# fnzhan/Neural-Gauge-Fields

Measured on AMD Instinct MI355X. Metric: Mray/sec (800x800 lego-style frame, 192 samples/ray), higher is better.
Workload: dtype f32; 1 GPU; TriPlane 800x800 frame, S=192, preset R1 (seeded random planes 256^2, dense density preset), gauge on, white_bg; samples_per_ray=192, bake_density=1, bake_color=1, launcher=none (single process)

## Files before the change

### neural-gauge-fields_amd/csrc/ngf_field.hip

```cpp
#include <map>
#include <mutex>
#include <utility>

#include "ngf_host.hpp"
#include "ngf_infoinv.hpp"
#include "ngf_pack.hpp"
#include "ngf_render.hpp"
#include "ngf_alpha.hpp"
#ifdef NGF_EXPERIMENTS
#include "ngf_render_pc.hpp"
#include "ngf_stage.hpp"
#endif

using namespace ngf;

static thread_local char g_err[512] = "";

int ngf::fail(int code, const char *fmt, ...)
{
    va_list ap;
    va_start(ap, fmt);
    vsnprintf(g_err, sizeof(g_err), fmt, ap);
    va_end(ap);
    return code;
}

static std::atomic<int> g_knob[ngf::KNOB_COUNT];
static const char *const g_knob_name[ngf::KNOB_COUNT] = {"tile_w", "split", "waves", "nstep", "profile", "ablate", "uv_tiles", "kernel", "stage", "poison", "grid", "xcd", "tail", "ord_rows", "ord_px", "train_dwg", "pairpack"};
static bool g_knob_init = [] { for (auto &k : g_knob) k.store(-1); return true; }();

int ngf::knob(int id) { return g_knob[id].load(std::memory_order_relaxed); }

hipError_t ngf::ensure_dynamic_lds(const void *kernel, size_t bytes)
{
    static std::mutex mu;
    static std::map<std::pair<int, const void *>, size_t> done;
    int dev = 0;
    hipError_t e = hipGetDevice(&dev);
    if (e != hipSuccess) return e;
    std::lock_guard<std::mutex> lock(mu);
    size_t &have = done[{dev, kernel}];
    if (have >= bytes && have != 0) return hipSuccess;
    e = hipFuncSetAttribute(kernel, hipFuncAttributeMaxDynamicSharedMemorySize, (int)bytes);
    if (e == hipSuccess) have = bytes;
    return e;
}

__global__ void __launch_bounds__(1024) dirty_lds_kernel(unsigned pattern, int words, int spin)
{
    extern __shared__ unsigned dirty_smem[];
    for (int i = threadIdx.x; i < words; i += blockDim.x) dirty_smem[i] = pattern;
    __syncthreads();
    const unsigned long long t0 = __builtin_readcyclecounter();
    while (__builtin_readcyclecounter() - t0 < (unsigned long long)spin) __builtin_amdgcn_s_sleep(8);
    if (dirty_smem[(threadIdx.x * 97) % words] != pattern) __builtin_trap();
}

int ngf::poison_lds(hipStream_t st)
{
    if (knob(KNOB_POISON) < 0 || !(knob(KNOB_POISON) & 1)) return NGF_OK;
    constexpr int kBytes = 160 * 1024;
    static int cus = 0;
    if (!cus) {
        int dev = 0;
        hipDeviceProp_t prop;
        HIP_TRY(hipGetDevice(&dev));
        HIP_TRY(hipGetDeviceProperties(&prop, dev));
        cus = prop.multiProcessorCount;
    }
    HIP_TRY(ensure_dynamic_lds(reinterpret_cast<const void *>(dirty_lds_kernel), kBytes));
    hipLaunchKernelGGL(dirty_lds_kernel, dim3(2 * cus), dim3(1024), kBytes, st, kPoisonPattern, kBytes / 4, 40000);
    HIP_TRY(hipGetLastError());
    return NGF_OK;
}

int ngf::poison_alloc(void *p, size_t bytes, hipStream_t st)
{
    if (knob(KNOB_POISON) < 0 || !(knob(KNOB_POISON) & 2) || !p) return NGF_OK;
    HIP_TRY(hipMemsetD32Async((hipDeviceptr_t)p, (int)kPoisonPattern, bytes / 4, st));
    return NGF_OK;
}

extern "C" int ngf_debug_dirty_lds(void *hip_stream)
{
    const int old = g_knob[ngf::KNOB_POISON].load();
    g_knob[ngf::KNOB_POISON].store(1);
    const int rc = ngf::poison_lds((hipStream_t)hip_stream);
    g_knob[ngf::KNOB_POISON].store(old);
    return rc;
}

__global__ void xcd_histogram_kernel(unsigned *out)
{
    if (threadIdx.x == 0) atomicAdd(out + xcd_id(), 1u);
    const unsigned long long t0 = __builtin_readcyclecounter();
    while (__builtin_readcyclecounter() - t0 < 20000ull) __builtin_amdgcn_s_sleep(8);
}
extern "C" int ngf_debug_xcd_histogram(unsigned *out8, int32_t workgroups, void *hip_stream)
{
    if (!out8 || workgroups <= 0) return fail(NGF_E_ARG, "ngf_debug_xcd_histogram: bad argument");
    HIP_TRY(hipMemsetAsync(out8, 0, 8 * sizeof(unsigned), (hipStream_t)hip_stream));
    hipLaunchKernelGGL(xcd_histogram_kernel, dim3(workgroups), dim3(768), 0, (hipStream_t)hip_stream, out8);
    HIP_TRY(hipGetLastError());
    return NGF_OK;
}

extern "C" int ngf_debug_set(const char *name, int32_t value)
{
    if (!name) return fail(NGF_E_ARG, "ngf_debug_set: null name");
    for (int k = 0; k < ngf::KNOB_COUNT; ++k)
        if (!strcmp(name, g_knob_name[k])) { g_knob[k].store(value); return NGF_OK; }
    return fail(NGF_E_ARG, "ngf_debug_set: unknown knob '%s'", name);
}

extern "C" int32_t ngf_debug_get(const char *name)
{
    if (name)
        for (int k = 0; k < ngf::KNOB_COUNT; ++k)
            if (!strcmp(name, g_knob_name[k])) return g_knob[k].load();
    return -1;
}

struct ngf_field {
    int32_t model = 0, flags = 0, plane_c = 0, dens_dim = 0, app = 0;
    float *tex[9] = {nullptr, nullptr, nullptr, nullptr, nullptr, nullptr, nullptr, nullptr, nullptr};
    float *blob = nullptr;
    float *basis_pack = nullptr;
    double *w1pd_tmp = nullptr;
    float *w1p_tmp = nullptr;
    uint8_t *mask = nullptr;
    uint8_t *mask_cells = nullptr;
    uint8_t *mask_any = nullptr, *mask_clear = nullptr, *mask_clear4 = nullptr;
    unsigned int *counters = nullptr;
    mutable std::atomic<unsigned> next_counter{0};
    RenderArgs proto;
    int64_t bytes = 0;
    int num_cus = 256;
    std::vector<std::pair<void *, size_t>> allocs;
    int dev = 0;
    mutable std::mutex use_mu;
    mutable std::vector<hipStream_t> streams;
    mutable std::atomic<void *> last_stream{(void *)(intptr_t)-1};
};

static inline void field_use(const ngf_field *f, hipStream_t st)
{
    if (f->last_stream.load(std::memory_order_relaxed) == (void *)st) return;
    std::lock_guard<std::mutex> lk(f->use_mu);
    bool known = false;
    for (hipStream_t s : f->streams) known |= s == st;
    if (!known) f->streams.push_back(st);
    f->last_stream.store((void *)st, std::memory_order_relaxed);
}

extern "C" int64_t ngf_debug_packed_plane_floats(int32_t H, int32_t W, int32_t nc, int32_t pair)
{
    if (H < 1 || W < 1 || nc < 1) return -1;
    return (int64_t)packed_plane_floats(H, W, nc, pair != 0);
}

template <int LOG>
__global__ void __launch_bounds__(64) mask_block_any_kernel(const uint8_t *__restrict__ cells, int D, int H, int W, int bH, int bW, uint8_t *__restrict__ any)
{
    constexpr int B = 1 << LOG;
    const int b = blockIdx.x, X = b % bW, Y = (b / bW) % bH, Z = b / (bW * bH);
    const int z = Z * B - 16 + ((int)threadIdx.x >> LOG), y = Y * B - 16 + ((int)threadIdx.x & (B - 1));
    unsigned acc = 0;
    if ((int)threadIdx.x < B * B && z >= 0 && z <= D && y >= 0 && y <= H) {
        const uint8_t *row = cells + ((size_t)z * (H + 1) + y) * (W + 1);
#pragma unroll
        for (int t = 0; t < B; ++t) {
            const int x = X * B - 16 + t;
            if (x >= 0 && x <= W) acc |= row[x];
        }
    }
    const unsigned long long m = __ballot(acc != 0);
    if (threadIdx.x == 0) any[b] = m ? 1 : 0;
}

__global__ void __launch_bounds__(256) mask_block_clear_kernel(const uint8_t *__restrict__ any, int cD, int cH, int cW, uint8_t *__restrict__ clear)
{
    const int b = blockIdx.x * blockDim.x + threadIdx.x;
    if (b >= cD * cH * cW) return;
    const int X = b % cW, Y = (b / cW) % cH, Z = b / (cW * cH);
    unsigned acc = 0;
    for (int dz = -1; dz <= 1; ++dz)
        for (int dy = -1; dy <= 1; ++dy)
            for (int dx = -1; dx <= 1; ++dx) {
                const int x = X + dx, y = Y + dy, z = Z + dz;
                if (x >= 0 && x < cW && y >= 0 && y < cH && z >= 0 && z < cD) acc |= any[(z * cH + y) * cW + x];
            }
    clear[b] = acc ? 0 : 1;
}

__global__ void bake_density_kernel(const float *__restrict__ src, int H, int W, int nc, const float *__restrict__ wd,
                                    float *__restrict__ dst, int pair)
{
    const size_t total = (size_t)(H + 2) * (W + 2);
    for (size_t i = (size_t)blockIdx.x * blockDim.x + threadIdx.x; i < total; i += (size_t)gridDim.x * blockDim.x) {
        const int x = (int)(i % (W + 2)), y = (int)(i / (W + 2));
        double v = 0.0;
        if (x >= 1 && x <= W && y >= 1 && y <= H)
// ... 744 lines not shown
{
    int64_t r[4] = {0, 0, 0, 0};
    int sh[4] = {0, 0, 0, 0};
    const int nseg = make_tile_plan(n, wide, resident, tail16 >= 0 ? tail16 : kTailDefault16, r, sh);
    for (int k = 0; k < 4; ++k) { seg_rays[k] = k < nseg ? r[k] : 0; seg_shift[k] = k < nseg ? sh[k] : 0; }
    return nseg;
}

template <typename K>
static int launch_render(K kernel, K kernel_split, K kernel_prod, const ngf_field *f, RenderArgs &A, int threads, size_t lds_bytes, hipStream_t st, int wide_tile)
{
    const unsigned slot = f->next_counter.fetch_add(1) % kCounters;
    A.tile_counter = f->counters + (size_t)slot * kQueueHeads;
    if (int rc = poison_lds(st)) return rc;
    const int waves = threads / kWave;
    const int cus = knob(KNOB_GRID) > 0 && knob(KNOB_GRID) < f->num_cus ? knob(KNOB_GRID) : f->num_cus;
    const int64_t resident = (int64_t)cus * waves;
    int64_t seg_rays[4] = {0, 0, 0, 0};
    int seg_shift[4] = {0, 0, 0, 0};
    int nseg = 1;
    bool split = kernel_split != nullptr;
    if (knob(KNOB_SPLIT) >= 0) split = knob(KNOB_SPLIT) != 0 && kernel_split;
    const int forced = knob(KNOB_TILE_W);
    auto shift_of = [](int w) { int sft = 0; while ((1 << sft) < w) ++sft; return sft; };
    if (forced >= 0 || !split) {
        int tw = forced >= 0 ? forced : 64;
        if (tw != 64 && tw != 32 && tw != 16 && tw != 8 && tw != 4 && tw != 2 && tw != 1) return fail(NGF_E_ARG, "knob tile_w must be 64, 32, 16, 8, 4, 2 or 1");
        if (knob(KNOB_SPLIT) < 0) split = tw < 64 && kernel_split;
        if (tw < 4 && !split) return fail(NGF_E_ARG, "tiles of 2 or 1 rays exist in the split kernel only");
        seg_rays[0] = A.n; seg_shift[0] = shift_of(tw);
    } else {
        nseg = make_tile_plan(A.n, wide_tile, resident, knob(KNOB_TAIL) >= 0 ? knob(KNOB_TAIL) : kTailDefault16, seg_rays, seg_shift);
    }
    A.tile_shift = seg_shift[0];
    A.tile_w = 1 << seg_shift[0];
    int64_t tiles = 0, ray0 = 0;
    for (int k = 0; k < 4; ++k) {
        const int sft = k < nseg ? seg_shift[k] : seg_shift[nseg - 1];
        const int64_t r = k < nseg ? seg_rays[k] : 0;
        A.seg_shift[k] = sft;
        A.seg_ray0[k] = ray0;
        tiles += (r + (1 << sft) - 1) >> sft;
        ray0 += r;
        if (k < 3) {
            if (tiles >= ((int64_t)1 << 32)) return fail(NGF_E_ARG, "render launch of %lld tiles: split the ray list", (long long)tiles);
            A.seg_end[k] = (uint32_t)tiles;
        }
    }
    {
        const int64_t row_w = A.ord_tpr;
        A.ord_n = A.ord_tpr = A.ord_bw = A.ord_bh = 0;
        const int sft0 = seg_shift[0];
        if (split && row_w > 0 && (row_w & ((1 << sft0) - 1)) == 0 && (seg_rays[0] >> sft0) < ((int64_t)1 << 31)) {
            const int64_t tpr = row_w >> sft0, rows = seg_rays[0] / row_w;
            int64_t bh = knob(KNOB_ORD_ROWS) > 0 ? knob(KNOB_ORD_ROWS) : 80;
            int64_t bw = (knob(KNOB_ORD_PX) > 0 ? knob(KNOB_ORD_PX) : 80) >> sft0;
            if (bw < 1) bw = 1;
            if (bw > tpr) bw = tpr;
            if (knob(KNOB_ORD_ROWS) != 0 && tpr > bw && rows >= 2 && bh >= 2) {
                if (bh > rows) bh = rows;
                A.ord_tpr = (uint32_t)tpr; A.ord_bw = (uint32_t)bw; A.ord_bh = (uint32_t)bh;
                A.ord_n = (uint32_t)((rows / bh) * bh * tpr);
            }
        }
    }
    K k = split ? kernel_split : kernel;
#if defined(NGF_EXP_DUMP) || defined(NGF_EXP_TIMELINE)
    if (split && kernel_prod) k = kernel_prod;
#else
    if (split && kernel_prod && !A.dbg_weight && !A.dbg_sigma && !A.stats && !A.skip_rgb && !A.ablate) k = kernel_prod;
#endif
    HIP_TRY(ensure_dynamic_lds(reinterpret_cast<const void *>(k), lds_bytes));
    if (tiles >= ((int64_t)1 << 32)) return fail(NGF_E_ARG, "render launch of %lld tiles: split the ray list", (long long)tiles);
    A.tiles = (uint32_t)tiles;
    A.xcd_queues = knob(KNOB_XCD) > 0 ? 8 : 1;
    int64_t grid = tiles < f->num_cus ? tiles : f->num_cus;
    if (knob(KNOB_GRID) > 0 && grid > knob(KNOB_GRID)) grid = knob(KNOB_GRID);
    if (grid < 1) grid = 1;
    const int64_t per_wg = (tiles + grid - 1) / grid;
    A.waves_active = per_wg < waves ? (int)per_wg : waves;
    A.queue_waves = (uint32_t)grid;
    hipLaunchKernelGGL(k, dim3((unsigned)grid), dim3(threads), lds_bytes, st, A);
    HIP_TRY(hipGetLastError());
    return NGF_OK;
}

template <typename P>
static int launch_policy(const ngf_field *f, RenderArgs &A, hipStream_t st)
{
    if constexpr (shared_gauge<P>::value) {
        if (!A.gauge_same) return launch_policy<GaugeAny<P>>(f, A, st);
    }
    const size_t lds = ((size_t)((A.blob_floats + 3) & ~3) + P::WAVES * wave_lds_floats<P>()) * sizeof(float);
    if (lds > 160 * 1024) return fail(NGF_E_ARG, "this waves-per-CU setting needs %zu bytes of LDS (> 160 KiB)", lds);
    constexpr int wide = P::INFOINV ? 16 : 8;
    using KP = decltype(&render_kernel<P, false>);
    if constexpr (P::NSTEP == 1 && P::PROD) return launch_render<KP>(render_kernel<P, false>, render_kernel<P, true>, render_kernel<P, true, false>, f, A, P::WAVES * kWave, lds, st, wide);
    else if constexpr (P::NSTEP == 1) return launch_render<KP>(render_kernel<P, false>, render_kernel<P, true>, nullptr, f, A, P::WAVES * kWave, lds, st, wide);
    else return launch_render<KP>(render_kernel<P, false>, nullptr, nullptr, f, A, P::WAVES * kWave, lds, st, wide);
}

#ifdef NGF_EXPERIMENTS
template <typename P, int NM, int NS, int TW>
static int launch_pc(const ngf_field *f, RenderArgs &A, hipStream_t st)
{
    if constexpr (shared_gauge<P>::value) {
        if (!A.gauge_same) return launch_pc<GaugeAny<P>, NM, NS, TW>(f, A, st);
    }
    const size_t lds = ((size_t)((A.blob_floats + 3) & ~3) + PcLds<NM>::TOTAL) * sizeof(float);
    if (lds > 160 * 1024) return fail(NGF_E_ARG, "the specialised kernel needs %zu bytes of LDS (> 160 KiB)", lds);
    const unsigned slot = f->next_counter.fetch_add(1) % kCounters;
    A.tile_counter = f->counters + (size_t)slot * kQueueHeads;
    HIP_TRY(hipMemsetAsync(A.tile_counter, 0, kQueueHeads * sizeof(unsigned), st));
    if (int rc = poison_lds(st)) return rc;
    A.xcd_queues = 1;
    A.tile_w = TW;
    A.tile_shift = TW == 8 ? 3 : 2;
    auto k = render_pc_kernel<P, NM, NS, TW>;
    HIP_TRY(ensure_dynamic_lds(reinterpret_cast<const void *>(k), lds));
    const int64_t tiles = (A.n + TW - 1) / TW;
    int64_t grid = (tiles + NM - 1) / NM;
    if (grid > f->num_cus) grid = f->num_cus;
    if (grid < 1) grid = 1;
    hipLaunchKernelGGL(k, dim3((unsigned)grid), dim3((NM + NS) * kWave), lds, st, A);
    HIP_TRY(hipMemsetAsync(A.tile_counter, 0, kQueueHeads * sizeof(unsigned), st));
    HIP_TRY(hipGetLastError());
    return NGF_OK;
}
#endif

template <bool BD, bool BC>
static int launch_triplane(const ngf_field *f, RenderArgs &A, hipStream_t st)
{
#ifndef NGF_EXPERIMENTS
    if (knob(KNOB_KERNEL) > 0 || knob(KNOB_STAGE) > 0 || knob(KNOB_PROFILE) > 0 || knob(KNOB_NSTEP) > 1 || (knob(KNOB_WAVES) >= 0 && knob(KNOB_WAVES) != 12))
        return fail(NGF_E_UNSUPPORTED, "knobs kernel / stage / profile / nstep / waves select experiment kernels: load libngf_hip_exp.so (built with -DNGF_EXPERIMENTS)");
    if constexpr (BD) {
        if (A.mask.coarse) return launch_policy<MaskSkip<TriPlanePolicy<BD, BC, 12, 1>>>(f, A, st);
    }
    return launch_policy<TriPlanePolicy<BD, BC, 12, 1>>(f, A, st);
#else
    int kernel = knob(KNOB_KERNEL) >= 0 ? knob(KNOB_KERNEL) : 0;
    if (A.dbg_weight || A.skip_rgb || knob(KNOB_NSTEP) > 1 || (knob(KNOB_PROFILE) > 0 && knob(KNOB_KERNEL) != 1)) kernel = 0;
    if (knob(KNOB_TILE_W) > 8 || knob(KNOB_SPLIT) == 0) kernel = 0;
    if (kernel == 1 && knob(KNOB_PROFILE) > 0) {
        if constexpr (!BC) {
            using PP = TriPlanePolicy<BD, false, 12, 1, true>;
            return knob(KNOB_WAVES) == 88 ? launch_pc<PP, 8, 8, 8>(f, A, st) : launch_pc<PP, 12, 4, 8>(f, A, st);
        }
    }
    if (kernel == 1) {
        using P = TriPlanePolicy<BD, BC, 12, 1>;
        int tw = A.n < 40 * (int64_t)f->num_cus * 12 ? 4 : 8;
        if (knob(KNOB_TILE_W) == 4 || knob(KNOB_TILE_W) == 8) tw = knob(KNOB_TILE_W);
        const int w = knob(KNOB_WAVES) >= 0 ? knob(KNOB_WAVES) : 124;
        switch (w) {
        case 124: return tw == 8 ? launch_pc<P, 12, 4, 8>(f, A, st) : launch_pc<P, 12, 4, 4>(f, A, st);
        case 88: return tw == 8 ? launch_pc<P, 8, 8, 8>(f, A, st) : launch_pc<P, 8, 8, 4>(f, A, st);
        case 84: return tw == 8 ? launch_pc<P, 8, 4, 8>(f, A, st) : launch_pc<P, 8, 4, 4>(f, A, st);
        case 128: return launch_pc<P, 12, 4, 8>(f, A, st);
        default: return fail(NGF_E_ARG, "specialised kernel: knob waves must be 124, 88 or 84");
        }
    }
    int w = 12, ns = 1;
    if (knob(KNOB_WAVES) >= 0) w = knob(KNOB_WAVES);
    if (knob(KNOB_NSTEP) >= 0) ns = knob(KNOB_NSTEP);
    if (ns == 2) {
        if (w == 8) return launch_policy<TriPlanePolicy<BD, BC, 8, 2>>(f, A, st);
        return fail(NGF_E_ARG, "knob nstep = 2 is built for waves = 8 only");
    }
    if (knob(KNOB_STAGE) > 0 && !A.dbg_weight && !A.skip_rgb) {
        if constexpr (!BD && !BC) {
            if (w == 8) return launch_policy<TriPlaneStagedPolicy<8>>(f, A, st);
            if (w == 12) return launch_policy<TriPlaneStagedPolicy<12>>(f, A, st);
            return fail(NGF_E_ARG, "knob stage: waves must be 8 (gauge + density strips) or 12 (gauge strips)");
        }
    }
    if (knob(KNOB_PROFILE) > 0) {
        if constexpr (!BC) return launch_policy<TriPlanePolicy<BD, false, 12, 1, true>>(f, A, st);
    }
    switch (w) {
    case 8: return launch_policy<TriPlanePolicy<BD, BC, 8, 1>>(f, A, st);
    case 12:
        if constexpr (BD) {
            if (A.mask.coarse) return launch_policy<MaskSkip<TriPlanePolicy<BD, BC, 12, 1>>>(f, A, st);
        }
        return launch_policy<TriPlanePolicy<BD, BC, 12, 1>>(f, A, st);
    case 16: return launch_policy<TriPlanePolicy<BD, BC, 16, 1>>(f, A, st);
    default: return fail(NGF_E_ARG, "knob waves must be 8, 12 or 16");
    }
#endif
}

static int render_common(const ngf_field *f, RenderArgs &A, hipStream_t st)
{
    field_use(f, st);
    if (f->model == NGF_MODEL_INFOINV) {
        const bool wide = knob(KNOB_TILE_W) > 16 || knob(KNOB_SPLIT) == 0;
        if (f->flags & NGF_F_SPLIT_BF16) {
            if (wide) return fail(NGF_E_ARG, "InfoInv NGF_F_SPLIT_BF16 renders with split tiles of at most 16 rays");
            return A.mask.coarse ? launch_policy<MaskSkip<InfoInvSplitPolicy>>(f, A, st) : launch_policy<InfoInvSplitPolicy>(f, A, st);
        }
        if (wide) return launch_policy<InfoInvWidePolicy>(f, A, st);
        return A.mask.coarse ? launch_policy<MaskSkip<InfoInvPolicy>>(f, A, st) : launch_policy<InfoInvPolicy>(f, A, st);
    }
    if (f->flags & NGF_F_NO_FOLD) return launch_policy<TriPlaneNoFoldPolicy>(f, A, st);
    if ((f->flags & NGF_F_SPLIT_BF16) && (f->flags & NGF_F_BAKE_COLOR)) return A.mask.coarse ? launch_policy<MaskSkip<TriPlaneBakedBf16Policy>>(f, A, st) : launch_policy<TriPlaneBakedBf16Policy>(f, A, st);
    if (f->flags & NGF_F_SPLIT_BF16) {
        if (knob(KNOB_TILE_W) > 8 || knob(KNOB_SPLIT) == 0) return fail(NGF_E_ARG, "NGF_F_SPLIT_BF16 renders with split tiles of 4 or 8 rays");
#ifdef NGF_EXPERIMENTS
        if (knob(KNOB_WAVES) == 12)
            return (f->flags & NGF_F_BAKE_DENSITY) ? launch_policy<TriPlaneBf16Policy<true, 12>>(f, A, st) : launch_policy<TriPlaneBf16Policy<false, 12>>(f, A, st);
#endif
        return (f->flags & NGF_F_BAKE_DENSITY) ? launch_policy<TriPlaneBf16Policy<true, 8>>(f, A, st) : launch_policy<TriPlaneBf16Policy<false, 8>>(f, A, st);
    }
    const bool bd = f->flags & NGF_F_BAKE_DENSITY, bc = f->flags & NGF_F_BAKE_COLOR;
    if (bd) return bc ? launch_triplane<true, true>(f, A, st) : launch_triplane<true, false>(f, A, st);
    return bc ? launch_triplane<false, true>(f, A, st) : launch_triplane<false, false>(f, A, st);
}

extern "C" int ngf_field_render(const ngf_field *f, const float *rays, int64_t n, int32_t n_samples, int32_t white_bg,
                                int32_t mode, const float *jitter, float *rgb, float *depth, uint64_t *stats, void *hip_stream)
{
    if (!f || !rays || !rgb || !depth) return fail(NGF_E_ARG, "ngf_field_render: null argument");
    if (n < 0 || n_samples <= 0) return fail(NGF_E_ARG, "ngf_field_render: n=%lld n_samples=%d", (long long)n, n_samples);
    if (n == 0) return NGF_OK;
    RenderArgs A = f->proto;
    A.rays = rays; A.jitter = jitter; A.rgb = rgb; A.depth = depth; A.n = n; A.S = n_samples;
    A.white_bg = white_bg ? 1 : 0; A.mode = mode ? 1 : 0; A.stats = (unsigned long long *)stats;
    if (knob(KNOB_ABLATE) > 0) A.ablate = knob(KNOB_ABLATE);
    return render_common(f, A, (hipStream_t)hip_stream);
}

extern "C" int ngf_field_render_image(const ngf_field *f, const float *rays, int64_t n, int32_t row_width, int32_t n_samples, int32_t white_bg,
                                      int32_t mode, const float *jitter, float *rgb, float *depth, uint64_t *stats, void *hip_stream)
{
    if (!f || !rays || !rgb || !depth) return fail(NGF_E_ARG, "ngf_field_render_image: null argument");
    if (n < 0 || n_samples <= 0) return fail(NGF_E_ARG, "ngf_field_render_image: n=%lld n_samples=%d", (long long)n, n_samples);
    if (n == 0) return NGF_OK;
    RenderArgs A = f->proto;
    A.rays = rays; A.jitter = jitter; A.rgb = rgb; A.depth = depth; A.n = n; A.S = n_samples;
    A.white_bg = white_bg ? 1 : 0; A.mode = mode ? 1 : 0; A.stats = (unsigned long long *)stats;
    if (knob(KNOB_ABLATE) > 0) A.ablate = knob(KNOB_ABLATE);
    A.ord_tpr = row_width > 0 && (int64_t)row_width < n && f->model == NGF_MODEL_TRIPLANE ? (uint32_t)row_width : 0u;
    return render_common(f, A, (hipStream_t)hip_stream);
}

extern "C" int ngf_field_march(const ngf_field *f, const float *rays, int64_t n, int32_t n_samples, int32_t mode,
                               const float *jitter, float *sigma, float *weight, void *hip_stream)
{
    if (!f || !rays || !sigma || !weight) return fail(NGF_E_ARG, "ngf_field_march: null argument");
    if (n <= 0 || n_samples <= 0) return fail(NGF_E_ARG, "ngf_field_march: n=%lld n_samples=%d", (long long)n, n_samples);
    hipStream_t st = (hipStream_t)hip_stream;
    float *scratch = nullptr;
    HIP_TRY(hipMallocAsync((void **)&scratch, (size_t)n * 4 * sizeof(float), st));
    RenderArgs A = f->proto;
    A.rays = rays; A.jitter = jitter; A.rgb = scratch; A.depth = scratch + 3 * n; A.n = n; A.S = n_samples;
    A.white_bg = 0; A.mode = mode ? 1 : 0; A.skip_rgb = 1; A.dbg_sigma = sigma; A.dbg_weight = weight;
    int rc = render_common(f, A, st);
    (void)hipFreeAsync(scratch, st);
    return rc;
}

extern "C" int ngf_field_decode_rgb(const ngf_field *f, const float *coords, const float *dirs, int64_t n, int32_t mode,
                                    float *rgb, void *hip_stream)
{
    if (!f || !coords || !dirs || !rgb) return fail(NGF_E_ARG, "ngf_field_decode_rgb: null argument");
    if (n <= 0) return fail(NGF_E_ARG, "ngf_field_decode_rgb: n=%lld", (long long)n);
    hipStream_t st = (hipStream_t)hip_stream;
    field_use(f, st);
// ... 130 lines not shown
```

### neural-gauge-fields_amd/csrc/ngf_render.hpp

```cpp
#pragma once
#include <cstddef>
#include <type_traits>

#include "ngf_device.hpp"
#include "ngf_shade16.hpp"
#include "ngf_shade_bf16.hpp"

namespace ngf {


template <typename P> constexpr int wave_lds_floats() { return P::RING * kRecFloats + P::BATCH * 4 + P::VFEAT_FLOATS + P::STAGE_FLOATS; }

__device__ __forceinline__ void view_inputs(const float d[3], float v[16])
{
    v[0] = d[0]; v[1] = d[1]; v[2] = d[2];
#pragma unroll
    for (int k = 0; k < 3; ++k) {
        sincos_small(d[k], v[3 + 2 * k], v[9 + 2 * k]);
        sincos_small(d[k] * 2.0f, v[4 + 2 * k], v[10 + 2 * k]);
    }
    v[15] = 0.0f;
}

__device__ __forceinline__ void view_inputs_tile(const float d[3], float *dst, int seg, int K)
// ... 60 lines not shown
        Bil b = bil_setup<BAKED>(t[2 * p], t[2 * p + 1], tx);
        if (cells) cells[p] = b;
        if (BAKED && PAIR) {
            const f32x4_a8 q = *tex_at<f32x4_a8>(tx.p, (uint32_t)b.idx * 2u);
            f += bil_mix(b, q[0], q[2], q[1], q[3]);
        } else if (BAKED) {
            const float *q = tex_at<float>(tx.p, (uint32_t)b.idx), *q1 = tex_at<float>(tx.p, (uint32_t)(b.idx + tx.stride));
            f += bil_mix(b, q[0], q[1], q1[0], q1[1]);
        } else {
            const f32x4 *q00 = tex_at<f32x4>(tx.p, (uint32_t)b.idx * 16u);
            const f32x4 *q01 = tex_at<f32x4>(tx.p, (uint32_t)(b.idx + tx.stride) * 16u);
            float d00 = 0.0f, d10 = 0.0f, d01 = 0.0f, d11 = 0.0f;
            typedef const __attribute__((address_space(4))) float *kptr_t;
            kptr_t wdp = (kptr_t)((const __attribute__((address_space(4))) char *)__builtin_amdgcn_kernarg_segment_ptr() + offsetof(RenderArgs, wd)) + p * 16;
            asm volatile("" : "+s"(wdp));
#pragma unroll
            for (int q = 0; q < 4; ++q) {
                f32x4 v00 = q00[q], v10 = q00[4 + q], v01 = q01[q], v11 = q01[4 + q];
#pragma unroll
                for (int e = 0; e < 4; ++e) {
                    float w = wdp[4 * q + e];
                    d00 = fmaf(w, v00[e], d00);
                    d10 = fmaf(w, v10[e], d10);
                    d01 = fmaf(w, v01[e], d01);
                    d11 = fmaf(w, v11[e], d11);
                }
            }
            f += bil_mix(b, d00, d10, d01, d11);
        }
    }
    return f + A.bd;
}

template <bool MED3 = true, bool PAIR = false, bool SAME = false>
__device__ __forceinline__ void triplane_gauge(const RenderArgs &A, const float x[3], int gauge_on, float t[6])
{
    const float u[3] = {x[0], x[1], x[0]}, v[3] = {x[1], x[2], x[2]};
    if (gauge_on) {
        float d[3][2];
        auto fetch = [&](int p, const Tex &tx, const Bil &b) {
            f32x2 g00, g10, g01, g11;
            if constexpr (PAIR) {
                const f32x4 *g = tex_at<f32x4>(tx.p, (uint32_t)b.idx * 4u);
                const f32x4 a = g[0], c = g[1];
                g00 = f32x2{a[0], a[1]}; g01 = f32x2{a[2], a[3]}; g10 = f32x2{c[0], c[1]}; g11 = f32x2{c[2], c[3]};
            } else {
                const f32x2 *g = tex_at<f32x2>(tx.p, (uint32_t)b.idx * 2u), *g1 = tex_at<f32x2>(tx.p, (uint32_t)(b.idx + tx.stride) * 2u);
                g00 = g[0]; g10 = g[1]; g01 = g1[0]; g11 = g1[1];
            }
            d[p][0] = bil_mix(b, g00[0], g10[0], g01[0], g11[0]);
            d[p][1] = bil_mix(b, g00[1], g10[1], g01[1], g11[1]);
        };
        if constexpr (PAIR && MED3 && SAME) {
            const Tex t0 = karg_tex(offsetof(RenderArgs, gau));
            BilAxis ax[3];
#pragma unroll
            for (int k = 0; k < 3; ++k) ax[k] = bil_axis(x[k], t0.fw);
            const int ua[3] = {0, 1, 0}, va[3] = {1, 2, 2};
#pragma unroll
            for (int p = 0; p < 3; ++p) {
                Tex tx = t0;
                tx.p = karg<const float *>(offsetof(RenderArgs, gau) + p * sizeof(Tex) + offsetof(Tex, p));
                fetch(p, tx, bil_from_axes(ax[ua[p]], ax[va[p]], t0.stride));
            }
        } else {
#pragma unroll
            for (int p = 0; p < 3; ++p) {
                const Tex tx = karg_tex(offsetof(RenderArgs, gau) + p * sizeof(Tex));
                fetch(p, tx, bil_setup<MED3>(u[p], v[p], tx));
            }
        }
        t[0] = (u[0] + d[0][0]) + d[2][0];  t[1] = (v[0] + d[0][1]) + d[1][0];
        t[2] = (u[1] + d[1][0]) + d[0][1];  t[3] = (v[1] + d[1][1]) + d[2][1];
        t[4] = (u[2] + d[2][0]) + d[0][0];  t[5] = (v[2] + d[2][1]) + d[1][1];
    } else {
#pragma unroll
        for (int p = 0; p < 3; ++p) { t[2 * p] = u[p]; t[2 * p + 1] = v[p]; }
    }
}

template <bool BAKE_D, bool BAKE_C, int WAVES_, int NSTEP_, bool PROFILE_ = false>
struct TriPlanePolicy {
    static constexpr bool PROFILE = PROFILE_;
    static constexpr bool PROD = WAVES_ == 12 && NSTEP_ == 1 && !PROFILE_;
    static constexpr bool INFOINV = false;
    static constexpr bool MASK_SKIP = false;
    static constexpr bool STAGED = false;
    static constexpr int STAGE_FLOATS = 0;
    static constexpr int WAVES = WAVES_;
    static constexpr int NSTEP = NSTEP_;
    static constexpr int BATCH = kBatch16;
    static constexpr bool VLDS = WAVES_ <= 12;
    static constexpr int VFEAT_FLOATS = VLDS ? kWave * kViewFeat : 0;
    static constexpr int RING = NSTEP_ == 1 ? 128 : 256;
    static constexpr bool REC12 = WAVES_ == 12 && NSTEP_ == 1 && !PROFILE_;
    static constexpr bool GATHER_QUAD = BAKE_C;
    static constexpr bool SHARED_GAUGE = BAKE_D;
    template <bool SAME>
    __device__ static __forceinline__ float sigma_impl(const RenderArgs &A, bool valid, const float x[3], float t[6], Bil *cells)
    {
        float tt[6];
        float f;
#ifdef NGF_EXPERIMENTS
        if (BAKE_D && !A.pairpack) {
            triplane_gauge<BAKE_D, false>(A, x, A.mode, tt);
            f = triplane_density_feature<BAKE_D, false>(A, tt, cells);
        } else
#endif
        {
            triplane_gauge<BAKE_D, BAKE_D, SAME>(A, x, A.mode, tt);
            f = triplane_density_feature<BAKE_D, BAKE_D>(A, tt, cells);
        }
        const float sg = softplus_shift(f);
#pragma unroll
        for (int k = 0; k < 6; ++k) t[k] = valid ? tt[k] : 0.0f;
        return valid ? sg : 0.0f;
    }
    __device__ static __forceinline__ float sigma(const RenderArgs &A, const float *, bool valid, const float x[3], int, float t[6], Bil *cells = nullptr)
    {
        return sigma_impl<true>(A, valid, x, t, cells);
    }
    static constexpr bool VIEW_FOLD = VLDS;
    __device__ static __forceinline__ void fold_view(const float *smem, const float *vfeat, float *pre, int n_rays, int lane)
    {
        if constexpr (BAKE_C) view_fold16<MlpLayout16Baked::W1V / 64, MlpLayout16Baked::B1, 4>(per_pass16(smem), vfeat, pre, n_rays, lane);
        else view_fold16<MlpLayout16<48>::W1 / 64 + 3 * MlpLayout16<48>::QCH, MlpLayout16<48>::B1, MlpLayout16<48>::KT>(per_pass16(smem), vfeat, pre, n_rays, lane);
    }
    __device__ static __forceinline__ void fold_view_regs(const float *smem, const f32x4 v, float *pre, int n_rays, int lane)
    {
        if constexpr (BAKE_C) view_fold16_regs<MlpLayout16Baked::W1V / 64, MlpLayout16Baked::B1, 4>(per_pass16(smem), v, pre, n_rays, lane);
        else view_fold16_regs<MlpLayout16<48>::W1 / 64 + 3 * MlpLayout16<48>::QCH, MlpLayout16<48>::B1, MlpLayout16<48>::KT>(per_pass16(smem), v, pre, n_rays, lane);
    }
    __device__ static __forceinline__ void shade(const RenderArgs &A, const float *smem, const float rec[kRecFloats], const float *vf,
                                                 const float od[3], int lane, float c[3], unsigned long long *tk = nullptr, const float *pre = nullptr)
    {
        f32x4 v = {0.0f, 0.0f, 0.0f, 0.0f};
        if (!pre) v = VLDS ? *reinterpret_cast<const f32x4 *>(vf + (lane >> 4) * 4) : view_entries16(od, lane >> 4);
        if constexpr (BAKE_C) mlp_pass16_baked(A, smem, rec, v, lane, c, pre);
        else mlp_pass16<48>(A, smem, rec, v, lane, c, tk, pre);
    }
    __device__ static __forceinline__ void shade12(const RenderArgs &A, const float *smem, const RecCells &cells, const float *vf, int lane, float c[3],
                                                   const float *pre)
    {
        const float rec[kRecFloats] = {0.0f, 0.0f, 0.0f, 0.0f, 0.0f, 0.0f, 0.0f, 0.0f};
        f32x4 v = {0.0f, 0.0f, 0.0f, 0.0f};
        if (!pre) v = *reinterpret_cast<const f32x4 *>(vf + (lane >> 4) * 4);
        if constexpr (BAKE_C) mlp_pass16_baked(A, smem, rec, v, lane, c, pre, &cells);
        else mlp_pass16<48>(A, smem, rec, v, lane, c, nullptr, pre, &cells);
    }
};

template <typename P>
struct MaskSkip : P {
#ifdef NGF_EXP_NO_MASK_SKIP
    static constexpr bool MASK_SKIP = false;
#else
    static constexpr bool MASK_SKIP = true;
#endif
};

template <typename P>
struct GaugeAny : P {
    static constexpr bool SHARED_GAUGE = false;
    __device__ static __forceinline__ float sigma(const RenderArgs &A, const float *, bool valid, const float x[3], int, float t[6], Bil *cells = nullptr)
    {
        return P::template sigma_impl<false>(A, valid, x, t, cells);
    }
};
template <typename P, typename = void> struct shared_gauge : std::false_type {};
template <typename P> struct shared_gauge<P, std::void_t<decltype(P::SHARED_GAUGE)>> : std::integral_constant<bool, P::SHARED_GAUGE> {};

template <bool BAKE_D, int WAVES_ = 8>
struct TriPlaneBf16Policy : TriPlanePolicy<BAKE_D, false, WAVES_, 1> {
    static constexpr bool PROD = WAVES_ == 8;
    static constexpr bool REC12 = false;
    static constexpr bool VIEW_FOLD = false;
    static constexpr int VFEAT_FLOATS = 8 * kViewFeat;
    __device__ static __forceinline__ void shade(const RenderArgs &A, const float *smem, const float rec[kRecFloats], const float *vf,
                                                 const float od[3], int lane, float c[3], unsigned long long * = nullptr, const float * = nullptr)
    {
        const f32x4 v = *reinterpret_cast<const f32x4 *>(vf + (lane >> 4) * 4);
        if constexpr (WAVES_ > 8) mlp_pass16_bf16_rows(A, smem, rec, v, lane, c);
        else mlp_pass16_bf16(A, smem, rec, v, lane, c);
    }
};

struct TriPlaneBakedBf16Policy : TriPlanePolicy<true, true, 12, 1> {
    using LB = MlpLayout16BakedBf16;
    __device__ static __forceinline__ void fold_view(const float *smem, const float *vfeat, float *pre, int n_rays, int lane)
    {
        view_fold16<LB::W1V / 64, LB::B1, 4>(per_pass16(smem), vfeat, pre, n_rays, lane);
    }
    __device__ static __forceinline__ void fold_view_regs(const float *smem, const f32x4 v, float *pre, int n_rays, int lane)
    {
        view_fold16_regs<LB::W1V / 64, LB::B1, 4>(per_pass16(smem), v, pre, n_rays, lane);
    }
    __device__ static __forceinline__ void shade(const RenderArgs &A, const float *smem, const float rec[kRecFloats], const float *vf,
                                                 const float od[3], int lane, float c[3], unsigned long long * = nullptr, const float *pre = nullptr)
    {
        f32x4 v = {0.0f, 0.0f, 0.0f, 0.0f};
        if (!pre) v = *reinterpret_cast<const f32x4 *>(vf + (lane >> 4) * 4);
        mlp_pass16_baked_bf16(A, smem, rec, v, lane, c, pre);
    }
    __device__ static __forceinline__ void shade12(const RenderArgs &A, const float *smem, const RecCells &cells, const float *vf, int lane, float c[3],
                                                   const float *pre)
    {
        const float rec[kRecFloats] = {0.0f, 0.0f, 0.0f, 0.0f, 0.0f, 0.0f, 0.0f, 0.0f};
        f32x4 v = {0.0f, 0.0f, 0.0f, 0.0f};
        if (!pre) v = *reinterpret_cast<const f32x4 *>(vf + (lane >> 4) * 4);
        mlp_pass16_baked_bf16(A, smem, rec, v, lane, c, pre, &cells);
    }
};

struct TriPlaneNoFoldPolicy : TriPlanePolicy<false, false, 8, 1> {
    static constexpr bool PROD = false;
    static constexpr bool REC12 = false;
    static constexpr bool VIEW_FOLD = false;
    __device__ static __forceinline__ void shade(const RenderArgs &A, const float *smem, const float rec[kRecFloats], const float *vf,
                                                 const float od[3], int lane, float c[3], unsigned long long * = nullptr, const float * = nullptr)
    {
        const f32x4 v = *reinterpret_cast<const f32x4 *>(vf + (lane >> 4) * 4);
        mlp_pass16_nofold(A, smem, rec, v, lane, c);
    }
};

#define NGF_STR2(x) #x
#define NGF_STR(x) NGF_STR2(x)
#define NGF_SPLIT_CHAIN(M)                                                                                                                        \
    template <> __device__ __forceinline__ void split_chain<M>(float alpha, float z, float &T, float &acc, float &dep, float &w)                    \
    {                                                                                                                                               \
// ... 527 lines not shown
```

### neural-gauge-fields_amd/csrc/ngf_shade16.hpp

```cpp
#pragma once
#include "ngf_device.hpp"

namespace ngf {

constexpr int kBatch16 = 16;
constexpr int kFoldStride = 68;

template <int APP>
struct MlpLayout16 {
    static constexpr int QCH = APP / 4;
    static constexpr int KT = 3 * QCH + 4;
    static constexpr int W1 = 0;
    static constexpr int W2 = W1 + 4 * KT * 64;
    static constexpr int B1 = W2 + 4 * 16 * 64;
    static constexpr int B2 = B1 + 64;
    static constexpr int W3 = B2 + 64;
    static constexpr int B3 = W3 + 192;
    static constexpr int TOTAL = B3 + 4;
};

struct MlpLayout16Baked {
    static constexpr int W1V = 0;
    static constexpr int W2 = W1V + 4 * 4 * 64;
    static constexpr int B1 = W2 + 4 * 16 * 64;
    static constexpr int B2 = B1 + 64;
    static constexpr int W3 = B2 + 64;
    static constexpr int B3 = W3 + 192;
    static constexpr int TOTAL = B3 + 4;
};

struct MlpLayout16BakedBf16 {
    static constexpr int W1V = 0;
    static constexpr int W2 = W1V + 4 * 4 * 64;
    static constexpr int B1 = W2 + 4 * 2 * 3 * 64 * 4;
    static constexpr int B2 = B1 + 64;
    static constexpr int W3 = B2 + 64;
    static constexpr int B3 = W3 + 192;
    static constexpr int TOTAL = B3 + 4;
};

__device__ __forceinline__ const float *per_pass16(const float *blob)
{
    int z = 0;
    asm volatile("" : "+v"(z));
    return blob + z;
}

__device__ __forceinline__ f32x4 view_entries16(const float d[3], int kq)
{
    f32x4 v;
#pragma unroll
    for (int e = 0; e < 4; ++e) {
        const int f = 4 * kq + e;
        const int g = f < 3 ? 0 : (f < 9 ? f - 3 : (f < 15 ? f - 9 : 0));
        const int dim = g >> 1;
        const float dd = dim == 0 ? d[0] : (dim == 1 ? d[1] : d[2]);
        float s, c;
        sincos_small((g & 1) ? dd * 2.0f : dd, s, c);
        const float raw = f == 0 ? d[0] : (f == 1 ? d[1] : d[2]);
        v[e] = f < 3 ? raw : (f < 9 ? s : (f < 15 ? c : 0.0f));
    }
    return v;
}

#define NGF_MFMA16(a, b, c) __builtin_amdgcn_mfma_f32_16x16x4f32((a), (b), (c), 0, 0, 0)

__device__ __forceinline__ float relu1(float x) { return __int_as_float(max(__float_as_int(x), 0)); }

__device__ __forceinline__ float sigmoid_rcp(float s) { return __builtin_amdgcn_rcpf(1.0f + expf(-s)); }

__device__ __forceinline__ void mlp_tail16(const float *blob, int oW2, int oB2, int oW3, int oB3, int lane, const f32x4 acc[4],
                                           float rgb[3], unsigned long long *tk = nullptr)
{
    const int kq = lane >> 4;
    f32x4 c[4];
#pragma unroll
    for (int mt = 0; mt < 4; ++mt) c[mt] = *reinterpret_cast<const f32x4 *>(blob + oB2 + kq * 16 + mt * 4);
    const float *w2 = blob + oW2 + lane;
#ifndef NGF_EXP_RELU_INTERLEAVED
    float h[16];
#pragma unroll
    for (int t = 0; t < 16; ++t) h[t] = relu1(acc[t >> 2][t & 3]);
    __builtin_amdgcn_sched_barrier(0);
// ... 310 lines not shown
    constexpr int H = ST & 1;
#ifndef NGF_PK_MIX
#pragma unroll
    for (int q = 0; q < 2; ++q)
#pragma unroll
        for (int e = 0; e < 4; ++e) {
            const int k = (2 * H + q) * 4 + e;
            const float s0 = ST < 2 ? 0.0f : sum[k >> 1][k & 1];
            sum[k >> 1][k & 1] = fmaf(g.wb[1], g.raw[3][q][e], fmaf(g.wb[0], g.raw[2][q][e], fmaf(g.wa[1], g.raw[1][q][e], fmaf(g.wa[0], g.raw[0][q][e], s0))));
        }
#else
#pragma unroll
    for (int tap = 0; tap < 4; ++tap)
#pragma unroll
        for (int q = 0; q < 2; ++q)
#pragma unroll
            for (int e = 0; e < 4; e += 2) {
                const int k = ((2 * H + q) * 4 + e) >> 1;
                const f32x2 t = {g.raw[tap][q][e], g.raw[tap][q][e + 1]};
                if (tap == 0) sum[k] = ST < 2 ? pk_mul_wlo(g.wa, t) : pk_fma_wlo(g.wa, t, sum[k]);
                else if (tap == 1) sum[k] = pk_fma_whi(g.wa, t, sum[k]);
                else if (tap == 2) sum[k] = pk_fma_wlo(g.wb, t, sum[k]);
                else sum[k] = pk_fma_whi(g.wb, t, sum[k]);
            }
#endif
}

template <typename L>
__device__ __forceinline__ void baked16_layer1(const RenderArgs &A, const float *blob, const float rec[kRecFloats], const f32x4 v,
                                               int lane, f32x4 acc[4], const float *pre, const RecCells *gcells)
{
    const int kq = lane >> 4;
    const int sg = lane >> 2, kqg = lane & 3;
    float rg[kRecFloats];
    rg[0] = rec[0]; rg[1] = rec[1];
    if (!gcells) {
#pragma unroll
        for (int k = 2; k < kRecFloats; ++k) rg[k] = __shfl(rec[k], sg);
    } else {
#pragma unroll
        for (int k = 2; k < kRecFloats; ++k) rg[k] = 0.0f;
    }
    BakedHalf ga, gb;
    baked16_issue<0>(A, rg, kqg, ga, gcells);
    __builtin_amdgcn_sched_barrier(0);
    baked16_issue<1>(A, rg, kqg, gb, gcells);
    __builtin_amdgcn_sched_barrier(0);
    f32x2 sum[8];
    baked16_consume<0>(ga, sum);
    __builtin_amdgcn_sched_barrier(0);
    baked16_issue<2>(A, rg, kqg, ga, gcells);
    __builtin_amdgcn_sched_barrier(0);
    baked16_consume<1>(gb, sum);
    __builtin_amdgcn_sched_barrier(0);
    baked16_issue<3>(A, rg, kqg, gb, gcells);
    __builtin_amdgcn_sched_barrier(0);
    baked16_consume<2>(ga, sum);
    __builtin_amdgcn_sched_barrier(0);
    baked16_issue<4>(A, rg, kqg, ga, gcells);
    __builtin_amdgcn_sched_barrier(0);
    baked16_consume<3>(gb, sum);
    __builtin_amdgcn_sched_barrier(0);
    baked16_issue<5>(A, rg, kqg, gb, gcells);
    __builtin_amdgcn_sched_barrier(0);
    baked16_consume<4>(ga, sum);
    __builtin_amdgcn_sched_barrier(0);
    baked16_consume<5>(gb, sum);
    __builtin_amdgcn_sched_barrier(0);
    const int src = 4 * (lane & 15) + kq;
    const float *b0 = pre ? pre + kq * 16 : blob + L::B1 + kq * 16;
#pragma unroll
    for (int mt = 0; mt < 4; ++mt)
#pragma unroll
        for (int e = 0; e < 4; ++e) acc[mt][e] = b0[4 * mt + e] + __shfl(sum[(4 * mt + e) >> 1][e & 1], src);
    if (!pre) {
        const float *w1 = blob + L::W1V + lane;
#pragma unroll
        for (int j = 0; j < 4; ++j)
#pragma unroll
            for (int mt = 0; mt < 4; ++mt) acc[mt] = NGF_MFMA16(w1[(mt * 4 + j) * 64], v[j], acc[mt]);
    }
}

__device__ __forceinline__ void mlp_pass16_baked(const RenderArgs &A, const float *blob, const float rec[kRecFloats], const f32x4 v,
                                                 int lane, float rgb[3], const float *pre = nullptr, const RecCells *gcells = nullptr)
{
    using L = MlpLayout16Baked;
    blob = per_pass16(blob);
    f32x4 acc[4];
    baked16_layer1<L>(A, blob, rec, v, lane, acc, pre, gcells);
    mlp_tail16(blob, L::W2, L::B2, L::W3, L::B3, lane, acc, rgb);
}

}
```

Measured before the change: 151.2 Mray/s.

## Add sixteen-wave production path with quarter-plane pipelined baked color gather

Adds a 16-waves-per-CU production policy for the baked density+color case, selected automatically when there are enough rays per CU and the LDS fits. The baked layer-1 color gather is split into quarter-plane stages with two or three buffers in flight, which lowers the number of live registers needed at 16 waves while keeping loads overlapped. This aims to raise occupancy and memory latency hiding. The risks are register spills, LDS pressure, and a different gather order that may hurt cache locality.

```diff
diff --git a/neural-gauge-fields_amd/csrc/ngf_field.hip b/neural-gauge-fields_amd/csrc/ngf_field.hip
--- a/neural-gauge-fields_amd/csrc/ngf_field.hip
+++ b/neural-gauge-fields_amd/csrc/ngf_field.hip
@@ -30,6 +30,7 @@
 static bool g_knob_init = [] { for (auto &k : g_knob) k.store(-1); return true; }();
 
 int ngf::knob(int id) { return g_knob[id].load(std::memory_order_relaxed); }
+static std::atomic<int> g_last_waves{-1};
 
 hipError_t ngf::ensure_dynamic_lds(const void *kernel, size_t bytes)
 {
@@ -118,6 +119,7 @@
     if (name)
         for (int k = 0; k < ngf::KNOB_COUNT; ++k)
             if (!strcmp(name, g_knob_name[k])) return g_knob[k].load();
+    if (name && !strcmp(name, "last_waves")) return g_last_waves.load();
     return -1;
 }
 
@@ -1028,6 +1030,7 @@
     A.queue_waves = (uint32_t)grid;
     hipLaunchKernelGGL(k, dim3((unsigned)grid), dim3(threads), lds_bytes, st, A);
     HIP_TRY(hipGetLastError());
+    g_last_waves.store(waves, std::memory_order_relaxed);
     return NGF_OK;
 }
 
@@ -1075,16 +1078,37 @@
 }
 #endif
 
+static constexpr int64_t kW16MinRaysPerCu = 312;
+static bool level3_waves16(const ngf_field *f, const RenderArgs &A)
+{
+    using P = TriPlanePolicy<true, true, 16, 1>;
+    static_assert(P::W16 && P::PROD && P::REC12 && P::VLDS && P::VIEW_FOLD, "the sixteen-wave level-3 policy is the production pass");
+    const size_t lds = ((size_t)((A.blob_floats + 3) & ~3) + P::WAVES * wave_lds_floats<P>()) * sizeof(float);
+    if (lds > 160 * 1024) return false;
+    if (knob(KNOB_WAVES) >= 0) return knob(KNOB_WAVES) == 16;
+    return A.n >= kW16MinRaysPerCu * f->num_cus;
+}
+
+template <bool BD, bool BC, int W>
+static int launch_fused(const ngf_field *f, RenderArgs &A, hipStream_t st)
+{
+    if constexpr (BD) {
+        if (A.mask.coarse) return launch_policy<MaskSkip<TriPlanePolicy<BD, BC, W, 1>>>(f, A, st);
+    }
+    return launch_policy<TriPlanePolicy<BD, BC, W, 1>>(f, A, st);
+}
+
 template <bool BD, bool BC>
 static int launch_triplane(const ngf_field *f, RenderArgs &A, hipStream_t st)
 {
 #ifndef NGF_EXPERIMENTS
-    if (knob(KNOB_KERNEL) > 0 || knob(KNOB_STAGE) > 0 || knob(KNOB_PROFILE) > 0 || knob(KNOB_NSTEP) > 1 || (knob(KNOB_WAVES) >= 0 && knob(KNOB_WAVES) != 12))
+    if (knob(KNOB_KERNEL) > 0 || knob(KNOB_STAGE) > 0 || knob(KNOB_PROFILE) > 0 || knob(KNOB_NSTEP) > 1 ||
+        (knob(KNOB_WAVES) >= 0 && knob(KNOB_WAVES) != 12 && !(BD && BC && knob(KNOB_WAVES) == 16)))
         return fail(NGF_E_UNSUPPORTED, "knobs kernel / stage / profile / nstep / waves select experiment kernels: load libngf_hip_exp.so (built with -DNGF_EXPERIMENTS)");
-    if constexpr (BD) {
-        if (A.mask.coarse) return launch_policy<MaskSkip<TriPlanePolicy<BD, BC, 12, 1>>>(f, A, st);
-    }
-    return launch_policy<TriPlanePolicy<BD, BC, 12, 1>>(f, A, st);
+    if constexpr (BD && BC) {
+        if (level3_waves16(f, A)) return launch_fused<BD, BC, 16>(f, A, st);
+    }
+    return launch_fused<BD, BC, 12>(f, A, st);
 #else
     int kernel = knob(KNOB_KERNEL) >= 0 ? knob(KNOB_KERNEL) : 0;
     if (A.dbg_weight || A.skip_rgb || knob(KNOB_NSTEP) > 1 || (knob(KNOB_PROFILE) > 0 && knob(KNOB_KERNEL) != 1)) kernel = 0;
@@ -1125,13 +1149,12 @@
     if (knob(KNOB_PROFILE) > 0) {
         if constexpr (!BC) return launch_policy<TriPlanePolicy<BD, false, 12, 1, true>>(f, A, st);
     }
+    if constexpr (BD && BC) {
+        if (w == 12 || w == 16) return level3_waves16(f, A) ? launch_fused<BD, BC, 16>(f, A, st) : launch_fused<BD, BC, 12>(f, A, st);
+    }
     switch (w) {
     case 8: return launch_policy<TriPlanePolicy<BD, BC, 8, 1>>(f, A, st);
-    case 12:
-        if constexpr (BD) {
-            if (A.mask.coarse) return launch_policy<MaskSkip<TriPlanePolicy<BD, BC, 12, 1>>>(f, A, st);
-        }
-        return launch_policy<TriPlanePolicy<BD, BC, 12, 1>>(f, A, st);
+    case 12: return launch_fused<BD, BC, 12>(f, A, st);
     case 16: return launch_policy<TriPlanePolicy<BD, BC, 16, 1>>(f, A, st);
     default: return fail(NGF_E_ARG, "knob waves must be 8, 12 or 16");
     }
diff --git a/neural-gauge-fields_amd/csrc/ngf_render.hpp b/neural-gauge-fields_amd/csrc/ngf_render.hpp
--- a/neural-gauge-fields_amd/csrc/ngf_render.hpp
+++ b/neural-gauge-fields_amd/csrc/ngf_render.hpp
@@ -166,7 +166,8 @@
 template <bool BAKE_D, bool BAKE_C, int WAVES_, int NSTEP_, bool PROFILE_ = false>
 struct TriPlanePolicy {
     static constexpr bool PROFILE = PROFILE_;
-    static constexpr bool PROD = WAVES_ == 12 && NSTEP_ == 1 && !PROFILE_;
+    static constexpr bool W16 = WAVES_ == 16 && BAKE_D && BAKE_C && NSTEP_ == 1 && !PROFILE_;
+    static constexpr bool PROD = (WAVES_ == 12 || W16) && NSTEP_ == 1 && !PROFILE_;
     static constexpr bool INFOINV = false;
     static constexpr bool MASK_SKIP = false;
     static constexpr bool STAGED = false;
@@ -174,10 +175,10 @@
     static constexpr int WAVES = WAVES_;
     static constexpr int NSTEP = NSTEP_;
     static constexpr int BATCH = kBatch16;
-    static constexpr bool VLDS = WAVES_ <= 12;
+    static constexpr bool VLDS = WAVES_ <= 12 || W16;
     static constexpr int VFEAT_FLOATS = VLDS ? kWave * kViewFeat : 0;
     static constexpr int RING = NSTEP_ == 1 ? 128 : 256;
-    static constexpr bool REC12 = WAVES_ == 12 && NSTEP_ == 1 && !PROFILE_;
+    static constexpr bool REC12 = (WAVES_ == 12 || W16) && NSTEP_ == 1 && !PROFILE_;
     static constexpr bool GATHER_QUAD = BAKE_C;
     static constexpr bool SHARED_GAUGE = BAKE_D;
     template <bool SAME>
@@ -220,7 +221,7 @@
     {
         f32x4 v = {0.0f, 0.0f, 0.0f, 0.0f};
         if (!pre) v = VLDS ? *reinterpret_cast<const f32x4 *>(vf + (lane >> 4) * 4) : view_entries16(od, lane >> 4);
-        if constexpr (BAKE_C) mlp_pass16_baked(A, smem, rec, v, lane, c, pre);
+        if constexpr (BAKE_C) mlp_pass16_baked<W16>(A, smem, rec, v, lane, c, pre);
         else mlp_pass16<48>(A, smem, rec, v, lane, c, tk, pre);
     }
     __device__ static __forceinline__ void shade12(const RenderArgs &A, const float *smem, const RecCells &cells, const float *vf, int lane, float c[3],
@@ -229,7 +230,7 @@
         const float rec[kRecFloats] = {0.0f, 0.0f, 0.0f, 0.0f, 0.0f, 0.0f, 0.0f, 0.0f};
         f32x4 v = {0.0f, 0.0f, 0.0f, 0.0f};
         if (!pre) v = *reinterpret_cast<const f32x4 *>(vf + (lane >> 4) * 4);
-        if constexpr (BAKE_C) mlp_pass16_baked(A, smem, rec, v, lane, c, pre, &cells);
+        if constexpr (BAKE_C) mlp_pass16_baked<W16>(A, smem, rec, v, lane, c, pre, &cells);
         else mlp_pass16<48>(A, smem, rec, v, lane, c, nullptr, pre, &cells);
     }
 };
diff --git a/neural-gauge-fields_amd/csrc/ngf_shade16.hpp b/neural-gauge-fields_amd/csrc/ngf_shade16.hpp
--- a/neural-gauge-fields_amd/csrc/ngf_shade16.hpp
+++ b/neural-gauge-fields_amd/csrc/ngf_shade16.hpp
@@ -1,4 +1,7 @@
 #pragma once
+#include <type_traits>
+#include <utility>
+
 #include "ngf_device.hpp"
 
 namespace ngf {
@@ -475,13 +478,126 @@
     }
 }
 
+#ifndef NGF_W16_STAGES
+#define NGF_W16_STAGES 2
+#endif
+
+struct BakedQuarter { f32x4 raw[4]; };
+
+__device__ __forceinline__ BilPk baked16_cell(const float rec[kRecFloats], int P, const Tex &t, const RecCells *cells)
+{
+    if (cells) return bil_from_rec_pk(cells->idx[P], cells->wx1[P], cells->wy1[P], (cells->bits >> (8 + P)) & 1);
+    const Bil b = bil_setup(rec[2 + 2 * P], rec[3 + 2 * P], t);
+    BilPk bp;
+    bp.idx = b.idx; bp.wa = f32x2{b.w00, b.w10}; bp.wb = f32x2{b.w01, b.w11};
+    return bp;
+}
+
+__device__ __forceinline__ void baked16q_issue(const float rec[kRecFloats], int st, int kq, BakedQuarter &g, const RecCells *cells)
+{
+    const int P = st >> 2, mt = st & 3;
+    const Tex t = karg_tex(offsetof(RenderArgs, app) + P * sizeof(Tex));
+    const int32_t idx = cells ? cells->idx[P] : baked16_cell(rec, P, t, cells).idx;
+    const f32x4 *t00 = tex_at<f32x4>(t.p, (uint32_t)idx * 64u + 4u * (kq + 4 * mt));
+    const f32x4 *t01 = tex_at<f32x4>(t.p, (uint32_t)(idx + t.stride) * 64u + 4u * (kq + 4 * mt));
+    g.raw[0] = t00[0];
+    g.raw[1] = t00[16];
+    g.raw[2] = t01[0];
+    g.raw[3] = t01[16];
+}
+
+__device__ __forceinline__ void baked16q_consume(const float rec[kRecFloats], int st, const BakedQuarter &g, f32x2 &wa, f32x2 &wb, f32x2 sum[8],
+                                                 const RecCells *cells)
+{
+    const int P = st >> 2, mt = st & 3;
+    if (mt == 0) {
+        const BilPk bp = baked16_cell(rec, P, cells ? Tex{} : karg_tex(offsetof(RenderArgs, app) + P * sizeof(Tex)), cells);
+        wa = bp.wa; wb = bp.wb;
+    }
+#pragma unroll
+    for (int e = 0; e < 4; ++e) {
+        const int k = mt * 4 + e;
+        const float s0 = P == 0 ? 0.0f : sum[k >> 1][k & 1];
+        sum[k >> 1][k & 1] = fmaf(wb[1], g.raw[3][e], fmaf(wb[0], g.raw[2][e], fmaf(wa[1], g.raw[1][e], fmaf(wa[0], g.raw[0][e], s0))));
+    }
+}
+
+template <int NB, int ST>
+__device__ __forceinline__ BakedQuarter &baked16q_buffer(BakedQuarter &g0, BakedQuarter &g1, BakedQuarter &g2)
+{
+    if constexpr (ST % NB == 0) return g0;
+    else if constexpr (ST % NB == 1) return g1;
+    else return g2;
+}
+template <int NB, int... ST>
+__device__ __forceinline__ void baked16q_stages(const float rg[kRecFloats], int kqg, BakedQuarter &g0, BakedQuarter &g1, BakedQuarter &g2, f32x2 sum[8],
+                                                const RecCells *gcells, std::integer_sequence<int, ST...>)
+{
+    f32x2 wa = {0.0f, 0.0f}, wb = {0.0f, 0.0f};
+    auto stage = [&](auto st_) {
+        constexpr int st = decltype(st_)::value;
+        BakedQuarter &g = baked16q_buffer<NB, st>(g0, g1, g2);
+        baked16q_consume(rg, st, g, wa, wb, sum, gcells);
+        __builtin_amdgcn_sched_barrier(0);
+        if constexpr (st + NB < 12) {
+            baked16q_issue(rg, st + NB, kqg, g, gcells);
+            __builtin_amdgcn_sched_barrier(0);
+        }
+    };
+    (stage(std::integral_constant<int, ST>{}), ...);
+}
+
+template <typename L, int NB = 2>
+__device__ __forceinline__ void baked16_layer1_quarters(const RenderArgs &A, const float *blob, const float rec[kRecFloats], const f32x4 v,
+                                                        int lane, f32x4 acc[4], const float *pre, const RecCells *gcells)
+{
+    static_assert(NB == 2 || NB == 3, "two or three quarter-plane stages in flight");
+    const int kq = lane >> 4;
+    const int sg = lane >> 2, kqg = lane & 3;
+    float rg[kRecFloats];
+    rg[0] = rec[0]; rg[1] = rec[1];
+    if (!gcells) {
+#pragma unroll
+        for (int k = 2; k < kRecFloats; ++k) rg[k] = __shfl(rec[k], sg);
+    } else {
+#pragma unroll
+        for (int k = 2; k < kRecFloats; ++k) rg[k] = 0.0f;
+    }
+    BakedQuarter g0, g1, g2;
+    baked16q_issue(rg, 0, kqg, g0, gcells);
+    __builtin_amdgcn_sched_barrier(0);
+    baked16q_issue(rg, 1, kqg, g1, gcells);
+    __builtin_amdgcn_sched_barrier(0);
+    if constexpr (NB == 3) {
+        baked16q_issue(rg, 2, kqg, g2, gcells);
+        __builtin_amdgcn_sched_barrier(0);
+    }
+    f32x2 sum[8];
+    baked16q_stages<NB>(rg, kqg, g0, g1, g2, sum, gcells, std::make_integer_sequence<int, 12>{});
+    const int src = 4 * (lane & 15) + kq;
+    const float *b0 = pre ? pre + kq * 16 : blob + L::B1 + kq * 16;
+#pragma unroll
+    for (int mt = 0; mt < 4; ++mt)
+#pragma unroll
+        for (int e = 0; e < 4; ++e) acc[mt][e] = b0[4 * mt + e] + __shfl(sum[(4 * mt + e) >> 1][e & 1], src);
+    if (!pre) {
+        const float *w1 = blob + L::W1V + lane;
+#pragma unroll
+        for (int j = 0; j < 4; ++j)
+#pragma unroll
+            for (int mt = 0; mt < 4; ++mt) acc[mt] = NGF_MFMA16(w1[(mt * 4 + j) * 64], v[j], acc[mt]);
+    }
+}
+
+template <bool QUARTER = false>
 __device__ __forceinline__ void mlp_pass16_baked(const RenderArgs &A, const float *blob, const float rec[kRecFloats], const f32x4 v,
                                                  int lane, float rgb[3], const float *pre = nullptr, const RecCells *gcells = nullptr)
 {
     using L = MlpLayout16Baked;
     blob = per_pass16(blob);
     f32x4 acc[4];
-    baked16_layer1<L>(A, blob, rec, v, lane, acc, pre, gcells);
+    if constexpr (QUARTER) baked16_layer1_quarters<L, NGF_W16_STAGES>(A, blob, rec, v, lane, acc, pre, gcells);
+    else baked16_layer1<L>(A, blob, rec, v, lane, acc, pre, gcells);
     mlp_tail16(blob, L::W2, L::B2, L::W3, L::B3, lane, acc, rgb);
 }
 
```

Result: faster. 159.7 Mray/s, median of 6 (+5.6%).
